# apple/ml-quant

Measured on AMD Instinct MI355X. Metric: images/sec ResNet-18 LS-1w/LS-2a 224x224 eval forward, higher is better.
Workload: dtype fp4 (e2m1, unit block scales) mfma on sign bits: exact integers in the f32 accumulator + f32; 1 GPU; ResNet-18 ImageNet ls-1 weight / ls-2 activation, synthetic 3x224x224, batch 256 per GPU, random-init weights; global_batch=256, parallelism=dp1 (batch-sharded replicas, RCCL all-gather of logits)

## Files before the change

### ml-quant_amd/csrc/lsq_pointwise.hip

```cpp

#include "lsq_common.h"

#ifdef LSQ_PW_SYNCTHREADS
#define PW_BARRIER() __syncthreads()
#else
#define PW_BARRIER() lds_barrier()
#endif
namespace lsq {
namespace {

typedef __attribute__((ext_vector_type(16))) float f32x16;

struct PwArgs {
  const float* x;
  const float* w;
  const float* bias;
  float* y;
  int N, C, H, W, O, Ho, Wo, s;
  long long P;
};

constexpr int kPitch = 68;

__global__ __launch_bounds__(256) void pointwise_conv_kernel(PwArgs a) {
  __shared__ __attribute__((aligned(16))) float ws[64][kPitch];
  __shared__ __attribute__((aligned(16))) float xs[64][kPitch];
  const int tid = threadIdx.x, lane = tid & 63, wid = tid >> 6;
  const unsigned n_ot = (unsigned)a.O >> 6;
  const long long p0 = (long long)(blockIdx.x / n_ot) * 64;
  const int o0 = (int)(blockIdx.x % n_ot) * 64;
  const int HoWo = a.Ho * a.Wo;
  const long long HW = (long long)a.H * a.W;
  const long long sp = min(p0 + lane, a.P - 1);
  const int sn = (int)(sp / HoWo);
  const int sr = (int)(sp - (long long)sn * HoWo);
  const int sho = sr / a.Wo, swo = sr - sho * a.Wo;
  const unsigned xoff = (unsigned)(((long long)sn * a.C + 16 * wid) * HW + (long long)sho * a.s * a.W + swo * a.s);
  const float* __restrict__ xsrc = a.x;
  const unsigned woff = (unsigned)(16 * wid * a.C + lane);
  const float* __restrict__ wsrc = a.w + (long long)o0 * a.C;
  const int mt = wid >> 1, nt = wid & 1;
  const int col = lane & 31, g = lane >> 5;
  f32x16 acc = {};
  float xv[16], wv[16];
#pragma unroll
  for (int i = 0; i < 16; ++i) xv[i] = (xsrc + (long long)i * HW)[xoff];
#pragma unroll
  for (int i = 0; i < 16; ++i) wv[i] = (wsrc + (long long)i * a.C)[woff];
  for (int c0 = 0; c0 < a.C; c0 += 64) {
    __syncthreads();
#pragma unroll
    for (int q = 0; q < 4; ++q)
      *reinterpret_cast<float4*>(&xs[lane][16 * wid + 4 * q]) = make_float4(xv[4 * q], xv[4 * q + 1], xv[4 * q + 2], xv[4 * q + 3]);
#pragma unroll
    for (int i = 0; i < 16; ++i) ws[16 * wid + i][lane] = wv[i];
    __syncthreads();
    if (c0 + 64 < a.C) {
#pragma unroll
      for (int i = 0; i < 16; ++i) xv[i] = (xsrc + (long long)(c0 + 64 + i) * HW)[xoff];
#pragma unroll
      for (int i = 0; i < 16; ++i) wv[i] = (wsrc + (long long)i * a.C + c0 + 64)[woff];
    }
#pragma unroll
    for (int h = 0; h < 2; ++h) {
      float4 af[4], bf[4];
#pragma unroll
      for (int q = 0; q < 4; ++q) {
        af[q] = *reinterpret_cast<const float4*>(&ws[mt * 32 + col][32 * g + 16 * h + 4 * q]);
        bf[q] = *reinterpret_cast<const float4*>(&xs[nt * 32 + col][32 * g + 16 * h + 4 * q]);
      }
#pragma unroll
      for (int q = 0; q < 4; ++q) {
        acc = __builtin_amdgcn_mfma_f32_32x32x2f32(af[q].x, bf[q].x, acc, 0, 0, 0);
        acc = __builtin_amdgcn_mfma_f32_32x32x2f32(af[q].y, bf[q].y, acc, 0, 0, 0);
        acc = __builtin_amdgcn_mfma_f32_32x32x2f32(af[q].z, bf[q].z, acc, 0, 0, 0);
        acc = __builtin_amdgcn_mfma_f32_32x32x2f32(af[q].w, bf[q].w, acc, 0, 0, 0);
      }
    }
  }
  const long long p = p0 + nt * 32 + col;
  const int ob = o0 + mt * 32 + 4 * g;
  float bv[16];
  if (a.bias) {
#pragma unroll
    for (int reg = 0; reg < 16; ++reg) bv[reg] = a.bias[ob + (reg & 3) + 8 * (reg >> 2)];
  } else {
#pragma unroll
    for (int reg = 0; reg < 16; ++reg) bv[reg] = 0.f;
  }
  if (p >= a.P) return;
  const int n = (int)(p / HoWo);
  const int r = (int)(p - (long long)n * HoWo);
  const unsigned yoff = (unsigned)(((long long)n * a.O + ob) * HoWo + r);
#pragma unroll
  for (int reg = 0; reg < 16; ++reg) (a.y + (long long)((reg & 3) + 8 * (reg >> 2)) * HoWo)[yoff] = acc[reg] + bv[reg];
}

typedef float f32x4 __attribute__((ext_vector_type(4)));

template <int NOT, bool PAIRS, bool VEC4>
__global__ __launch_bounds__(256) void pointwise_all_kernel(PwArgs a) {
  __shared__ __attribute__((aligned(16))) float ws[2][64][kPitch];
  __shared__ __attribute__((aligned(16))) float xs[64][kPitch];
  const int tid = threadIdx.x, lane = tid & 63, wid = tid >> 6;
  const long long p0 = (long long)blockIdx.x * 64;
  const int ob = (int)blockIdx.y * (NOT * 64);
  const int HoWo = a.Ho * a.Wo;
  const long long HW = (long long)a.H * a.W;
  const float* __restrict__ xsrc = a.x;
  unsigned xoff;
  if constexpr (PAIRS) {
    const long long sp = min(p0 + 2 * (tid & 31), a.P - 2);
    const int sn = (int)(sp / HoWo);
    const int sr = (int)(sp - (long long)sn * HoWo);
    const int sho = sr / a.Wo, swo = sr - sho * a.Wo;
    xoff = (unsigned)(((long long)sn * a.C + 8 * (tid >> 5)) * HW + (long long)sho * a.s * a.W + swo * a.s);
  } else {
    const long long sp = min(p0 + lane, a.P - 1);
    const int sn = (int)(sp / HoWo);
    const int sr = (int)(sp - (long long)sn * HoWo);
    const int sho = sr / a.Wo, swo = sr - sho * a.Wo;
    xoff = (unsigned)(((long long)sn * a.C + 16 * wid) * HW + (long long)sho * a.s * a.W + swo * a.s);
  }
  const unsigned woff = (unsigned)((tid >> 4) * a.C + 4 * (tid & 15));
  const int mt = wid >> 1, nt = wid & 1;
  const int col = lane & 31, g = lane >> 5;
  f32x16 acc[NOT];
#pragma unroll
  for (int t = 0; t < NOT; ++t)
#pragma unroll
    for (int q = 0; q < 16; ++q) acc[t][q] = 0.f;

  f32x4 xq[8];
  float xv[16];
  auto load_x = [&](int c0) {
    if constexpr (PAIRS) {
#pragma unroll
      for (int i = 0; i < 8; ++i) xq[i] = *reinterpret_cast<const f32x4*>(xsrc + (long long)(c0 + i) * HW + xoff);
    } else {
#pragma unroll
      for (int i = 0; i < 16; ++i) xv[i] = (xsrc + (long long)(c0 + i) * HW)[xoff];
    }
  };
  auto store_x = [&]() {
    if constexpr (PAIRS) {
      const int px = 2 * (tid & 31), cb = 8 * (tid >> 5);
      *reinterpret_cast<float4*>(&xs[px][cb]) = make_float4(xq[0][0], xq[1][0], xq[2][0], xq[3][0]);
      *reinterpret_cast<float4*>(&xs[px][cb + 4]) = make_float4(xq[4][0], xq[5][0], xq[6][0], xq[7][0]);
      *reinterpret_cast<float4*>(&xs[px + 1][cb]) = make_float4(xq[0][2], xq[1][2], xq[2][2], xq[3][2]);
      *reinterpret_cast<float4*>(&xs[px + 1][cb + 4]) = make_float4(xq[4][2], xq[5][2], xq[6][2], xq[7][2]);
    } else {
#pragma unroll
      for (int q = 0; q < 4; ++q)
        *reinterpret_cast<float4*>(&xs[lane][16 * wid + 4 * q]) = make_float4(xv[4 * q], xv[4 * q + 1], xv[4 * q + 2], xv[4 * q + 3]);
    }
  };
  f32x4 wq[4];
  auto load_w = [&](int t, int c0) {
    const float* wsrc = a.w + (long long)(ob + t * 64) * a.C + c0;
#pragma unroll
    for (int k = 0; k < 4; ++k) wq[k] = *reinterpret_cast<const f32x4*>(wsrc + (long long)(16 * k) * a.C + woff);
  };
  auto store_w = [&](int buf) {
#pragma unroll
    for (int k = 0; k < 4; ++k)
      *reinterpret_cast<float4*>(&ws[buf][(tid >> 4) + 16 * k][4 * (tid & 15)]) = make_float4(wq[k][0], wq[k][1], wq[k][2], wq[k][3]);
  };

  const int nchunks = a.C >> 6;
  load_x(0);
  load_w(0, 0);
  int buf = 0;
  for (int cc = 0; cc < nchunks; ++cc) {
    PW_BARRIER();
    store_x();
    if (cc + 1 < nchunks) load_x(64 * (cc + 1));
#pragma unroll
    for (int t = 0; t < NOT; ++t) {
      store_w(buf);
      PW_BARRIER();
      if (t + 1 < NOT) load_w(t + 1, 64 * cc);
      else if (cc + 1 < nchunks) load_w(0, 64 * (cc + 1));
#pragma unroll
      for (int h = 0; h < 2; ++h) {
        float4 af[4], bf[4];
#pragma unroll
        for (int q = 0; q < 4; ++q) {
          af[q] = *reinterpret_cast<const float4*>(&ws[buf][mt * 32 + col][32 * g + 16 * h + 4 * q]);
          bf[q] = *reinterpret_cast<const float4*>(&xs[nt * 32 + col][32 * g + 16 * h + 4 * q]);
        }
#pragma unroll
        for (int q = 0; q < 4; ++q) {
          acc[t] = __builtin_amdgcn_mfma_f32_32x32x2f32(bf[q].x, af[q].x, acc[t], 0, 0, 0);
          acc[t] = __builtin_amdgcn_mfma_f32_32x32x2f32(bf[q].y, af[q].y, acc[t], 0, 0, 0);
          acc[t] = __builtin_amdgcn_mfma_f32_32x32x2f32(bf[q].z, af[q].z, acc[t], 0, 0, 0);
          acc[t] = __builtin_amdgcn_mfma_f32_32x32x2f32(bf[q].w, af[q].w, acc[t], 0, 0, 0);
        }
      }
      buf ^= 1;
    }
  }
#pragma unroll
  for (int t = 0; t < NOT; ++t) {
    const int o = ob + 64 * t + mt * 32 + col;
    const float b = a.bias ? a.bias[o] : 0.f;
#pragma unroll
    for (int rg = 0; rg < 4; ++rg) {
      const long long p = p0 + nt * 32 + 8 * rg + 4 * g;
      if constexpr (VEC4) {
        if (p < a.P) {
          const int n = (int)(p / HoWo);
          const int r = (int)(p - (long long)n * HoWo);
          const f32x4 v = {acc[t][4 * rg] + b, acc[t][4 * rg + 1] + b, acc[t][4 * rg + 2] + b, acc[t][4 * rg + 3] + b};
          *reinterpret_cast<f32x4*>(a.y + ((long long)n * a.O + o) * HoWo + r) = v;
        }
      } else {
#pragma unroll
        for (int k = 0; k < 4; ++k) {
          const long long pk = p + k;
          if (pk < a.P) {
            const int n = (int)(pk / HoWo);
            const int r = (int)(pk - (long long)n * HoWo);
            a.y[((long long)n * a.O + o) * HoWo + r] = acc[t][4 * rg + k] + b;
          }
        }
      }
    }
  }
}

template <int NOT>
void launch_all(const PwArgs& a, dim3 grid, hipStream_t st) {
  const bool vec4 = ((a.Ho * a.Wo) & 3) == 0;
  if (a.s == 2 && (a.Wo & 1) == 0 && a.P >= 2) {
    if (vec4) hipLaunchKernelGGL((pointwise_all_kernel<NOT, true, true>), grid, dim3(256), 0, st, a);
    else hipLaunchKernelGGL((pointwise_all_kernel<NOT, true, false>), grid, dim3(256), 0, st, a);
  } else {
    if (vec4) hipLaunchKernelGGL((pointwise_all_kernel<NOT, false, true>), grid, dim3(256), 0, st, a);
    else hipLaunchKernelGGL((pointwise_all_kernel<NOT, false, false>), grid, dim3(256), 0, st, a);
  }
}

}
}

using namespace lsq;

extern "C" int lsq_pointwise_conv(const float* x, int N, int C, int H, int W, const float* w, const float* bias, int O,
                                  int stride, float* y, void* stream) {
  if (!x || !w || !y) return LSQ_E_NULL;
  if (N <= 0 || C <= 0 || H <= 0 || W <= 0 || O <= 0 || stride <= 0) return LSQ_E_SHAPE;
  if (C % 64 || O % 64) return LSQ_E_UNSUPPORTED;
  if ((long long)N * C * H * W >= (1ll << 30) || (long long)N * O * ((H - 1) / stride + 1) * ((W - 1) / stride + 1) >= (1ll << 30))
    return LSQ_E_UNSUPPORTED;
  PwArgs a = {};
  a.x = x; a.w = w; a.bias = bias; a.y = y;
  a.N = N; a.C = C; a.H = H; a.W = W; a.O = O; a.s = stride;
  a.Ho = (H - 1) / stride + 1;
  a.Wo = (W - 1) / stride + 1;
  a.P = (long long)N * a.Ho * a.Wo;
  const long long blocks = (a.P + 63) / 64;
  if (blocks * (O / 64) > 0x7FFFFFFF) return LSQ_E_SHAPE;
  const int n_ot = O / 64;
  const bool pair_ok = stride != 2 || (a.Wo & 1) || (W & 1) == 0;
  if (n_ot <= 8 && (n_ot & (n_ot - 1)) == 0 && pair_ok) {
    int per_wg = n_ot;
    long long min_wgs = 256;
#ifdef LSQ_TUNE
    if (const char* e = getenv("LSQ_PW_MINWG")) min_wgs = atoll(e);
#endif
    while (per_wg > 1 && blocks * (n_ot / per_wg) < min_wgs) per_wg >>= 1;
    const dim3 grid((unsigned)blocks, (unsigned)(n_ot / per_wg));
    switch (per_wg) {
      case 1: launch_all<1>(a, grid, (hipStream_t)stream); break;
      case 2: launch_all<2>(a, grid, (hipStream_t)stream); break;
      case 4: launch_all<4>(a, grid, (hipStream_t)stream); break;
      default: launch_all<8>(a, grid, (hipStream_t)stream); break;
    }
    return (int)hipGetLastError();
  }
  hipLaunchKernelGGL(pointwise_conv_kernel, dim3((unsigned)(blocks * (O / 64))), dim3(256), 0, (hipStream_t)stream, a);
  return (int)hipGetLastError();
}
```

Measured before the change: 123,200 images/sec.

## Stage pointwise conv epilogue through LDS for coalesced output stores

The epilogue of the fused pointwise kernel now writes accumulators (with bias) into a shared-memory tile, reusing the weight and input buffers as three slots, then re-reads them so each lane stores contiguous pixels along the output row. The goal is to replace the scattered per-lane global stores with coalesced float4 or scalar stores along the spatial dimension. In exchange it adds extra LDS traffic and barriers per group of output tiles. Optional cycle-counter instrumentation, enabled only by a compile-time macro, is also added.

Result: no change. 123,200 images/sec (-0.1%).

```diff
diff --git a/ml-quant_amd/csrc/lsq_pointwise.hip b/ml-quant_amd/csrc/lsq_pointwise.hip
--- a/ml-quant_amd/csrc/lsq_pointwise.hip
+++ b/ml-quant_amd/csrc/lsq_pointwise.hip
@@ -5,6 +5,32 @@
 #define PW_BARRIER() __syncthreads()
 #else
 #define PW_BARRIER() lds_barrier()
+#endif
+#ifdef LSQ_PW_CLOCKS
+constexpr int kPwClocks = 64;
+#define PW_CLK_INIT()                       \
+  __shared__ long long clk_s[kPwClocks];    \
+  int nclk = 0;                             \
+  const bool clk_on = threadIdx.x == 0 && blockIdx.x == gridDim.x / 2 && blockIdx.y == 0
+#define PW_CLK()                                                                                   \
+  do {                                                                                             \
+    __builtin_amdgcn_sched_barrier(0);                                                             \
+    if (clk_on && nclk < kPwClocks) clk_s[nclk++] = (long long)__builtin_readcyclecounter();       \
+    __builtin_amdgcn_sched_barrier(0);                                                             \
+  } while (0)
+#define PW_CLK_FLUSH()                                                                             \
+  do {                                                                                             \
+    asm volatile("s_waitcnt vmcnt(0)" ::: "memory");  \
+    PW_CLK();                                                                                      \
+    if (clk_on) {                                                                                  \
+      long long* dst = reinterpret_cast<long long*>(a.y + (long long)a.N * a.O * HoWo);            \
+      for (int i = 0; i < kPwClocks; ++i) dst[i] = i < nclk ? clk_s[i] : 0;                        \
+    }                                                                                              \
+  } while (0)
+#else
+#define PW_CLK_INIT() do {} while (0)
+#define PW_CLK() do {} while (0)
+#define PW_CLK_FLUSH() do {} while (0)
 #endif
 namespace lsq {
 namespace {
@@ -21,6 +47,7 @@
 };
 
 constexpr int kPitch = 68;
+constexpr int kSlots = 3;
 
 __global__ __launch_bounds__(256) void pointwise_conv_kernel(PwArgs a) {
   __shared__ __attribute__((aligned(16))) float ws[64][kPitch];
@@ -100,9 +127,11 @@
 
 template <int NOT, bool PAIRS, bool VEC4>
 __global__ __launch_bounds__(256) void pointwise_all_kernel(PwArgs a) {
-  __shared__ __attribute__((aligned(16))) float ws[2][64][kPitch];
-  __shared__ __attribute__((aligned(16))) float xs[64][kPitch];
+  __shared__ __attribute__((aligned(16))) float lds[kSlots][64][kPitch];
+  float (*const ws)[64][kPitch] = lds;
+  float (*const xs)[kPitch] = lds[2];
   const int tid = threadIdx.x, lane = tid & 63, wid = tid >> 6;
+  PW_CLK_INIT();
   const long long p0 = (long long)blockIdx.x * 64;
   const int ob = (int)blockIdx.y * (NOT * 64);
   const int HoWo = a.Ho * a.Wo;
@@ -168,17 +197,22 @@
   };
 
   const int nchunks = a.C >> 6;
+  PW_CLK();
   load_x(0);
   load_w(0, 0);
+  PW_CLK();
   int buf = 0;
   for (int cc = 0; cc < nchunks; ++cc) {
     PW_BARRIER();
+    PW_CLK();
     store_x();
     if (cc + 1 < nchunks) load_x(64 * (cc + 1));
+    PW_CLK();
 #pragma unroll
     for (int t = 0; t < NOT; ++t) {
       store_w(buf);
       PW_BARRIER();
+      PW_CLK();
       if (t + 1 < NOT) load_w(t + 1, 64 * cc);
       else if (cc + 1 < nchunks) load_w(0, 64 * (cc + 1));
 #pragma unroll
@@ -198,35 +232,60 @@
         }
       }
       buf ^= 1;
-    }
-  }
-#pragma unroll
-  for (int t = 0; t < NOT; ++t) {
-    const int o = ob + 64 * t + mt * 32 + col;
-    const float b = a.bias ? a.bias[o] : 0.f;
-#pragma unroll
-    for (int rg = 0; rg < 4; ++rg) {
-      const long long p = p0 + nt * 32 + 8 * rg + 4 * g;
-      if constexpr (VEC4) {
-        if (p < a.P) {
-          const int n = (int)(p / HoWo);
-          const int r = (int)(p - (long long)n * HoWo);
-          const f32x4 v = {acc[t][4 * rg] + b, acc[t][4 * rg + 1] + b, acc[t][4 * rg + 2] + b, acc[t][4 * rg + 3] + b};
-          *reinterpret_cast<f32x4*>(a.y + ((long long)n * a.O + o) * HoWo + r) = v;
-        }
-      } else {
-#pragma unroll
-        for (int k = 0; k < 4; ++k) {
-          const long long pk = p + k;
-          if (pk < a.P) {
-            const int n = (int)(pk / HoWo);
-            const int r = (int)(pk - (long long)n * HoWo);
-            a.y[((long long)n * a.O + o) * HoWo + r] = acc[t][4 * rg + k] + b;
+      PW_CLK();
+    }
+  }
+  PW_CLK();
+  const int spx = VEC4 ? 4 * (lane & 15) : lane;
+  const long long sp = p0 + spx;
+  const bool sp_ok = sp < a.P;
+  const long long spc = sp_ok ? sp : 0;
+  const int sn = (int)(spc / HoWo);
+  const int sr = (int)(spc - (long long)sn * HoWo);
+  float* __restrict__ ydst = a.y + ((long long)sn * a.O + ob) * HoWo + sr;
+  float bv[NOT];
+#pragma unroll
+  for (int t = 0; t < NOT; ++t) bv[t] = a.bias ? a.bias[ob + 64 * t + mt * 32 + col] : 0.f;
+#pragma unroll
+  for (int t0 = 0; t0 < NOT; t0 += kSlots) {
+    PW_BARRIER();
+#pragma unroll
+    for (int tt = 0; tt < kSlots; ++tt) {
+      const int t = t0 + tt;
+      if (t < NOT) {
+        const float b = bv[t];
+#pragma unroll
+        for (int rg = 0; rg < 4; ++rg)
+          *reinterpret_cast<float4*>(&lds[tt][mt * 32 + col][nt * 32 + 8 * rg + 4 * g]) =
+              make_float4(acc[t][4 * rg] + b, acc[t][4 * rg + 1] + b, acc[t][4 * rg + 2] + b, acc[t][4 * rg + 3] + b);
+      }
+    }
+    PW_BARRIER();
+    PW_CLK();
+#pragma unroll
+    for (int tt = 0; tt < kSlots; ++tt) {
+      const int t = t0 + tt;
+      if (t < NOT) {
+        if constexpr (VEC4) {
+#pragma unroll
+          for (int j = 0; j < 4; ++j) {
+            const int row = 16 * wid + 4 * j + (lane >> 4);
+            const float4 v = *reinterpret_cast<const float4*>(&lds[tt][row][spx]);
+            if (sp_ok) *reinterpret_cast<f32x4*>(ydst + (long long)(64 * t + row) * HoWo) = f32x4{v.x, v.y, v.z, v.w};
+          }
+        } else {
+#pragma unroll
+          for (int j = 0; j < 16; ++j) {
+            const int row = 16 * wid + j;
+            const float v = lds[tt][row][spx];
+            if (sp_ok) ydst[(long long)(64 * t + row) * HoWo] = v;
           }
         }
       }
     }
-  }
+    PW_CLK();
+  }
+  PW_CLK_FLUSH();
 }
 
 template <int NOT>
```
